# boolsi/boolsi

Hardware: AMD Instinct MI355X
Metric: node-state-updates/s (higher is better)
Workload: dtype u32

## Files before the change

boolsi_amd/csrc/bsx_cascade.cpp:

```cpp
#include <cmath>
#include <cstdio>
#include <cstring>

#include "bsx_attract_host.h"

using namespace bsx;

namespace {
constexpr uint64_t kUnresCap = 1ull << 16;
constexpr uint64_t kNearBytes = 1ull << 32;
}

namespace bsx {

static int mirror_slots_for(bsx_handle h, uint32_t* slots_out) {
    const uint64_t entries = (h->cube_mirror ? 2 : 1) * h->journal_states;
    uint32_t slots = 64;
    while (slots < 2 * entries && slots < h->cache_lds_slots) slots *= 2;
    const size_t fixed = h->shmem + 32 + pool_extra_bytes(h->net.nw);
    while (slots < 4 * entries && slots < h->cache_lds_slots && fixed + (size_t)2 * slots * h->cache_stride <= 80 * 1024) slots *= 2;
    h->mirror_slots = *slots_out = std::min(slots, h->cache_lds_slots);
    if (h->knobs.debug) std::fprintf(stderr, "[bsx] mirror: %llu cycle states cached, %u slots\n", (unsigned long long)h->journal_states, *slots_out);
    return BSX_OK;
}

int lean_mirror_slots(bsx_handle h, uint32_t* slots_out, Totals* tot) {
    uint32_t ignored = 0;
    if (!slots_out) slots_out = &ignored;
    if (!h->journal_stale) return mirror_slots_for(h, slots_out);
    unsigned int known = 0;
    HIPCHK(h, hipMemcpy(&known, h->d_cc_count.p, sizeof(known), hipMemcpyDeviceToHost));
    if (tot) ++tot->syncs;
    known = std::min<unsigned int>(known, kCycleJournalCap);
    h->h_journal.resize(known);
    if (known) HIPCHK(h, hipMemcpy(h->h_journal.data(), h->d_cc_journal.p, known * sizeof(CycleRecord), hipMemcpyDeviceToHost));
    uint64_t states = 0;
    uint32_t taken = 0;
    for (const CycleRecord& r : h->h_journal) {
        if (taken >= (uint32_t)kTagAcc + kLdsAcc) break;
        if (!r.ready || r.length == 0 || r.length > kCycleCacheMaxLen) continue;
        states += r.length;
        ++taken;
    }
    h->journal_states = states;
    h->journal_stale = false;
    return mirror_slots_for(h, slots_out);
}

int ensure_mirror_image(bsx_handle h, AttractParams& P, size_t shmem) {
    if (!h->knobs.mirror_image) { P.mirror_image = nullptr; P.mirror_out = nullptr; return BSX_OK; }
    const size_t words = 4 + (size_t)P.cc.lds_slots * (h->cache_stride / 4);
    if (h->image_n != h->h_journal.size() || h->image_slots != P.cc.lds_slots || h->d_mirror.n < words) {
        HIPCHK(h, h->d_mirror.reserve(words));
        AttractParams B = P;
        B.count = 0;
        B.level_in = nullptr;
        B.mirror_image = nullptr;
        B.mirror_out = h->d_mirror.p;
        HIPCHK(h, launch_attract_pool((int)h->net.nw, (int)h->net.k_mux, h->lut_mode, dim3(1), shmem, h->stream, B));
        h->image_n = h->h_journal.size();
        h->image_slots = P.cc.lds_slots;
    }
    P.mirror_image = h->d_mirror.p;
    P.mirror_out = nullptr;
    return BSX_OK;
}

}

namespace {

int order_cube_digits(bsx_handle h, Cube& c) {
    const uint32_t r = (uint32_t)c.rel.size();
    if (r < 2 || r > 64 || !h->knobs.cube_order) return BSX_OK;
    uint64_t need = 0;
    for (uint32_t q = 0; q < r; ++q) need |= 1ull << c.rel[q];
    if (need & ~h->life_valid) {
        LifetimeParams L{};
        L.net = h->net;
        for (int w = 0; w < kMaxW32; ++w) { L.fixmask[w] = h->sp.fixmask[w]; L.fixval[w] = h->sp.fixval[w]; L.base[w] = c.base[w]; L.free_mask[w] = c.free_mask[w]; }
        L.n_digits = r;
        for (uint32_t q = 0; q < r; ++q) L.node[q] = h->model.any[c.rel[q]];
        HIPCHK(h, h->d_life.reserve(64));
        HIPCHK(h, hipMemsetAsync(h->d_life.p, 0, 64 * sizeof(uint32_t), h->stream));
// ... 201 lines not shown
            }
        }
        const size_t shmem_here = Q.lower_build ? h->shmem + (size_t)B.slots * h->cache_stride + 32 + pool_lower_extra_bytes(nw) : B.shmem;
        hipStream_t const st = i == 0 ? main_st : tail_st;
        HIPCHK(h, launch_attract_pool((int)nw, (int)h->net.k_mux, h->lut_mode, grid, shmem_here, st, Q));
        if (i == 0) HIPCHK(h, hipEventRecord(ev[1], main_st));
        if (i == 0 && side) HIPCHK(h, hipStreamWaitEvent(tail_st, ev[1], 0));
    }
    if (side) {
        HIPCHK(h, hipEventRecord(ev[2], tail_st));
        slot_busy[slot] = ev[2];
    }
    return BSX_OK;
}

int evaluate_chain(bsx_handle h, const CascadeEnv& env, const CascadeShape& sh, const Chain& ch, MergedTable& pass_table,
                   u128& pass_none, u128& pass_ref, int& verdict, uint32_t& lower_to) {
    const AttractParams& P = env.P;
    Totals& tot = env.tot;
    const uint64_t max_t = env.max_t, max_len = env.max_len;
    const uint32_t nw = h->net.nw, rec_words = nw + 3;
    verdict = kChainOk;
    uint64_t n_entries = 0;
    for (uint32_t i = 0; i < ch.top; ++i) {
        const ChainLevel& l = ch.lv[i];
        const Counters& c = h->ctr_seen[ch.ctr_base + i];
        const uint64_t classes = i == 0 ? 1ull << l.k_bits : n_entries << l.k_bits;
        if (i > 0 && n_entries == 0) break;
        tot.steps_exec += c.steps_exec;
        if (h->knobs.debug)
            std::fprintf(stderr, "[bsx] cube 2^%u (%u digits free) at digit value %llu%s: depth %u%s, %u digits here (%u relevant), %llu classes, %llu near a cycle, %llu unresolved\n",
                         ch.c1.a, ch.c1.n_free, (unsigned long long)ch.c1.d_lo, ch.c1.fix_mask ? " [sub-block]" : "", l.depth, i == 0 ? " (top)" : l.per_parent ? " (per parent)" : "", l.k_bits, l.r_here,
                         (unsigned long long)classes, (unsigned long long)c.near_classes, (unsigned long long)c.straggler_classes);
        if (h->knobs.debug && l.per_parent) {
            const LeafProgram& prog = h->h_leaf[ch.index];
            std::fprintf(stderr, "[bsx] per-parent level: kb %u, %u enumerated rules, %u free rules, m %u\n", prog.kb, prog.n_enum, prog.n_free, prog.m);
        }
        if (c.straggler_overflow) { verdict = kChainGiveUp; return BSX_OK; }
        if (c.near_overflow) { verdict = kChainLower; lower_to = l.depth - 1; return BSX_OK; }
        n_entries = c.near_classes;
        {
            double* seen = h->plan.near_seen[i == 0 ? 0 : 1][std::min<uint32_t>(l.depth, kMaxCubeLevels)];
            seen[0] += (double)classes; seen[1] += (double)c.near_classes;
        }
        const uint32_t us = l.unit_shift;
        merge_cube_counters(pass_table, c, us, nw);
        fold_cube_level(c, us, max_t, pass_none, pass_ref);
        const uint64_t n_unres = c.straggler_classes;
        if (!n_unres) continue;
        if (n_unres > kUnresCap) { verdict = kChainGiveUp; return BSX_OK; }
        std::vector<uint32_t> recs(n_unres * rec_words);
        HIPCHK(h, hipMemcpy(recs.data(), h->d_unres.p + (size_t)(ch.ctr_base + i) * kUnresCap * rec_words, recs.size() * 4, hipMemcpyDeviceToHost));
        ++tot.syncs;
        std::vector<uint32_t> st(n_unres * nw);
        for (uint64_t q = 0; q < n_unres; ++q) std::copy(recs.begin() + q * rec_words, recs.begin() + q * rec_words + nw, st.begin() + q * nw);
        DevBuf<uint32_t> d_states;
        DevBuf<ProblemRec32> d_res;
        HIPCHK(h, d_states.upload(st));
        HIPCHK(h, d_res.alloc(n_unres));
        AttractParams S = P;
        S.sp = l.cube.sp;
        S.sp.tp_origin = 0;
        S.count = n_unres;
        S.states = d_states.p;
        S.per_problem = d_res.p;
        S.max_len = BSX_T_INF;
// ... 244 lines not shown
```

boolsi_amd/csrc/bsx_device.h:

```cpp
#pragma once
#include <cstddef>
#include <stdint.h>

namespace bsx {

constexpr int kWave = 64;
constexpr int kBlock = 512;
constexpr int kWavesPerBlock = kBlock / kWave;
constexpr int kPoolBlockThreads = 768;
constexpr uint32_t kPoolCap = 112;
constexpr uint32_t kPoolSlots = 128;
constexpr uint32_t pool_rec_words(uint32_t nw) { return nw + 4; }
constexpr uint32_t kLowerFoundWords = 256;
constexpr int kMaxW32 = 8;
constexpr int kMaxMuxK = 6;
constexpr int kTableSlots = 64;
constexpr uint32_t kStepLimit = 1u << 30;
constexpr uint64_t kDigestSeed = 0xCBF29CE484222325ull;
constexpr uint64_t kDigestPrime = 0x100000001B3ull;
constexpr uint32_t kMaxDepositRuns = 64;

struct DevNet {
    uint32_t n_nodes;
    uint32_t nw;
// ... 45 lines not shown
    uint32_t trajectory_l;
    uint32_t found;
    uint32_t pad;
};

struct alignas(256) Counters {
    unsigned long long cursor;
    unsigned long long steps_ref;
    unsigned long long steps_exec;
    unsigned long long n_none;
    unsigned long long log_cursor;
    unsigned int log_overflow;
    unsigned int step_limit_hits;
    unsigned long long n_stragglers;
    unsigned long long n_cache_resolved;
    unsigned long long straggler_classes;
    unsigned int straggler_overflow;
    unsigned int pad;
    unsigned long long table_inserts;
    unsigned int table_overflow;
    unsigned int near_overflow;
    unsigned long long phase_sum[3];
    unsigned long long phase_max[3];
    unsigned long long acc_cnt[64], acc_sl[64], acc_sl2_lo[64], acc_sl2_hi[64];
    unsigned int acc_len[64];
    unsigned int acc_key[64][kMaxW32];
    unsigned long long fix_cnt[64], fix_sl[64], fix_sl2[64];
    unsigned long long fix_none, fix_ref, fix_capfail;
    unsigned long long near_classes;
    unsigned long long t_first_not, t_last;
    unsigned long long wave_iters;
    unsigned long long service_rounds;
    unsigned long long diag[4];
};

constexpr uint32_t kCycleCacheMaxLen = 64;
constexpr uint32_t kCycleCacheLdsBytes = 16 * 1024;
constexpr uint32_t kCycleJournalCap = 4096;
constexpr uint32_t kCycleClaimSlots = 8192;
constexpr int kTagAcc = 3;
constexpr uint32_t kLdsAcc = 61;
constexpr uint32_t kMergeGroup = 32;
constexpr uint32_t kMergeSlots = 256;
constexpr uint32_t lean_acc_bytes(uint32_t nw) { return (kTagAcc + kLdsAcc) * (8 + 8 + 4 + 4 + 4 * nw) + 16 + kWavesPerBlock * (kMergeSlots + 256); }

struct CycleRecord {
    uint32_t key[kMaxW32];
    uint32_t length;
    uint32_t ready;
};
static_assert(sizeof(CycleRecord) == 40, "CycleRecord layout");

struct CycleCache {
    CycleRecord* journal;
    unsigned int* journal_count;
    unsigned int* claims;
    uint32_t enabled;
    uint32_t lds_slots;
};

struct LevelDesc {
    unsigned long long n_entries;
    unsigned int abort;
    unsigned int pad;
};
constexpr uint32_t kMaxCubeLevels = 16;
constexpr uint32_t kSideStreams = 4;
constexpr uint32_t kMaxChains = 48;
constexpr uint32_t kMaxChainBlocks = 160;
constexpr size_t kLevelDescBytes = 3584;
constexpr size_t kPublishTicketOffset = kLevelDescBytes - 16;
static_assert(sizeof(LevelDesc) * (kMaxChainBlocks + kMaxChains + 1) <= kPublishTicketOffset && kLevelDescBytes % 256 == 0, "descriptor block");

constexpr uint32_t kLeafMaxDeps = 64;
// ... 147 lines not shown
```

boolsi_amd/csrc/bsx_kernels_common.h:

```cpp
#pragma once
#include <hip/hip_runtime.h>
#include <type_traits>
#include "bsx_device.h"

namespace bsx {

__device__ __forceinline__ uint32_t bfi(uint32_t sel, uint32_t a, uint32_t b) {
    uint32_t r;
    asm("v_bfi_b32 %0, %1, %2, %3" : "=v"(r) : "v"(sel), "v"(a), "v"(b));
    return r;
}

#define BSX_KERNARG(Type, name)                                                                          \
    const Type* name = (const Type*)__builtin_amdgcn_kernarg_segment_ptr();                              \
    asm volatile("" : "+s"(name))

__device__ __forceinline__ uint32_t rank_below(uint64_t mask) {
    return __builtin_amdgcn_mbcnt_hi((uint32_t)(mask >> 32), __builtin_amdgcn_mbcnt_lo((uint32_t)mask, 0u));
}

template <int NW>
__device__ __forceinline__ bool eq_words(const uint32_t (&a)[NW], const uint32_t (&b)[NW]) {
    uint32_t d = 0;
#pragma unroll
// ... 285 lines not shown
        if (range == 3) { digit = (uint32_t)(variant % 3); variant /= 3; }
        else { digit = (uint32_t)(variant & 1); variant >>= 1; }
        const int st = digit_state(range, digit);
        if (st >= 0) { put_bit<NW>(pr.fm, node, 1); put_bit<NW>(pr.fv, node, (uint32_t)st); }
    }
    pr.pv_digits = 0;
    pr.tp = sp.tp_origin;
    for (uint32_t j = 0; j < sp.n_pv; ++j) {
        const uint32_t t = sp.pv[3 * j], range = sp.pv[3 * j + 2];
        uint32_t digit;
        if (range == 3) { digit = (uint32_t)(variant % 3); variant /= 3; }
        else { digit = (uint32_t)(variant & 1); variant >>= 1; }
        pr.pv_digits |= (uint64_t)digit << (2 * j);
        if (digit_state(range, digit) >= 0 && t > pr.tp) pr.tp = t;
    }
}

template <int NW>
__device__ __forceinline__ void apply_perturbations(const DevSpace& sp, uint32_t t, uint64_t pv_digits,
                                                    uint32_t (&s)[NW]) {
    if (t <= sp.tp_origin) {
#pragma unroll
        for (int w = 0; w < NW; ++w)
            s[w] = (s[w] & ~sp.sched_clr[t * NW + w]) | sp.sched_set[t * NW + w];
    }
    for (uint32_t j = 0; j < sp.n_pv; ++j) {
        if (sp.pv[3 * j] == t) {
            const int st = digit_state(sp.pv[3 * j + 2], (uint32_t)(pv_digits >> (2 * j)) & 3u);
            if (st >= 0) put_bit<NW>(s, sp.pv[3 * j + 1], (uint32_t)st);
        }
    }
}

template <int NW, int K, int LM>
__device__ __forceinline__ NetView<NW, K, LM> stage_network(const DevNet& net, uint32_t* smem, uint32_t*& smem_free) {
    constexpr bool LDS_LUT = LM != kLutGlobal;
    NetView<NW, K, LM> nv;
    if constexpr (LDS_LUT) {
        if ((uint32_t)(uintptr_t)(__attribute__((address_space(3))) uint32_t*)smem != 0u) __builtin_trap();
    }
    uint32_t* p = smem;
    uint32_t* smasks = p;
    const uint32_t n_masks = (1u << K) * NW;
    for (uint32_t i = threadIdx.x; i < n_masks; i += blockDim.x) smasks[i] = net.masks[i];
    p += (n_masks + 3u) & ~3u;
    if (LDS_LUT) {
        uint32_t* slut = p;
        const uint4* src = reinterpret_cast<const uint4*>(net.lut);
        uint4* dst = reinterpret_cast<uint4*>(slut);
        const uint32_t n4 = net.lut_words >> 2;
        for (uint32_t i = threadIdx.x; i < n4; i += blockDim.x) dst[i] = src[i];
        p += net.lut_words;
        nv.lut = slut;
    } else {
        nv.lut = net.lut;
    }
    __syncthreads();
    nv.masks = smasks;
    if constexpr (NetView<NW, K, LM>::kMasksInRegs) {
#pragma unroll
        for (int i = 0; i < (1 << K) * NW; ++i) nv.mreg[i] = smasks[i];
    } else {
        nv.mreg[0] = 0;
    }
    nv.n_wide = net.n_wide;
    nv.wide_desc = net.wide_desc;
    nv.wide_preds = net.wide_preds;
    nv.wide_tt = net.wide_tt;
    smem_free = p;
    return nv;
}

__device__ __forceinline__ uint32_t digest_ybit(uint32_t t) { return (t * 0x9E3779B1u) >> 31; }
template <int NW>
__device__ __forceinline__ uint64_t digest_fold_words(uint64_t dg, const uint32_t (&s)[NW], uint32_t w64) {
#pragma unroll
    for (int w = 0; w < (NW + 1) / 2; ++w) {
        uint64_t word = s[2 * w];
        if (2 * w + 1 < NW) word |= (uint64_t)s[2 * w + 1] << 32;
        if ((uint32_t)w < w64) dg = (dg ^ word) * kDigestPrime;
    }
    return dg;
}

__device__ __forceinline__ uint64_t bcast64(uint64_t v, int src_lane) {
    const uint32_t lo = __builtin_amdgcn_readlane((uint32_t)v, src_lane);
    const uint32_t hi = __builtin_amdgcn_readlane((uint32_t)(v >> 32), src_lane);
    return ((uint64_t)hi << 32) | lo;
}

__device__ __forceinline__ unsigned long long wave_sum(unsigned long long v) {
#pragma unroll
    for (int off = 32; off >= 1; off >>= 1) {
        const uint32_t lo = __shfl_xor((uint32_t)v, off, 64);
        const uint32_t hi = __shfl_xor((uint32_t)(v >> 32), off, 64);
        v += ((unsigned long long)hi << 32) | lo;
    }
    return v;
}
__device__ __forceinline__ void wave_atomic_add(unsigned long long* dst, unsigned long long v, int lane) {
    const unsigned long long total = wave_sum(v);
    if (lane == 0 && total) atomicAdd(dst, total);
// ... 342 lines not shown
```

boolsi_amd/csrc/bsx_pool_kernel.h:

```cpp
#pragma once
#include "bsx_kernels_common.h"
#include "bsx_leaf.h"

namespace bsx {

constexpr int kPoolBlock = kPoolBlockThreads;
constexpr int kPoolWaves = kPoolBlock / 64;
constexpr uint32_t kPoolGroup = 64;

constexpr int pool_min_waves(int nw) { return nw <= 2 ? 6 : 2; }

#define BSX_RARE_PARAMS(name) BSX_KERNARG(AttractParams, name)

template <int NW>
__device__ __forceinline__ void deposit_runs(const DevSpace& sp, uint64_t d, uint32_t (&s)[NW], uint32_t run_first = 0,
                                             uint32_t run_end = 0xFFFFFFFFu) {
    const uint32_t end = run_end < sp.n_runs ? run_end : sp.n_runs;
    for (uint32_t r = run_first; r < end; ++r) {
        const uint32_t desc = sp.deposit[2 * r], mask = sp.deposit[2 * r + 1];
        const uint32_t piece = ((uint32_t)(d >> (desc & 63u)) & mask) << ((desc >> 16) & 31u);
        const uint32_t word = (desc >> 8) & 7u;
#pragma unroll
        for (int w = 0; w < NW; ++w) s[w] |= (word == (uint32_t)w) ? piece : 0u;
    }
}

template <int NW, int K, int LM, bool CUBE, bool LOWER = false>
__global__ __launch_bounds__(kPoolBlock, pool_min_waves(NW)) void k_attract_pool(const AttractParams P) {
    static_assert(CUBE || !LOWER, "the lower-level build is a cube build");
    extern __shared__ __attribute__((aligned(16))) uint32_t smem[];
    uint32_t* smem_free;
#ifdef BSX_DIAG
    const unsigned long long dbg_t0 = wall_clock64();
#endif
    uint64_t n_items = P.count, chunk_first = P.chunk_first;
    uint32_t chunk = P.chunk;
    if constexpr (CUBE) {
        if (P.level_in) {
            const unsigned long long listed = P.level_in->n_entries;
            n_items = P.level_in->abort ? 0ull : listed << P.entry_shift;
            if constexpr (LOWER) {
                if (P.leaf && n_items) n_items = ((listed + 63ull) & ~63ull) * leaf_parts(P.leaf->m, listed, (uint64_t)gridDim.x * kPoolWaves);
            }
            if (n_items == 0) return;
            const uint64_t n_waves = (uint64_t)gridDim.x * kPoolWaves;
            if (n_items < (1ull << 28)) { chunk_first = ((n_items + n_waves - 1) / n_waves + 63) / 64 * 64; chunk = 0; }
            else { chunk_first = 4096; chunk = 4096; }
            if ((uint64_t)blockIdx.x * chunk_first >= n_items) return;
        }
    }
    if constexpr (CUBE) {
        if (threadIdx.x == 0 && !P.mirror_out) atomicMax(&P.ctr->t_first_not, ~(unsigned long long)wall_clock64());
    }
    const NetView<NW, K, LM> nv = stage_network<NW, K, LM>(P.net, smem, smem_free);
    const uint32_t lane = threadIdx.x & 63, wave = __builtin_amdgcn_readfirstlane(threadIdx.x >> 6);
    const uint32_t tp = P.sp.tp_origin;
    const bool has_warmup = tp != 0;
    const bool counting = CUBE || P.merge >= 2;
    constexpr bool cube = CUBE;
    const int32_t fast_steps = (int32_t)P.fast_steps;
    const uint32_t cmask = P.cc.lds_slots - 1;
    constexpr int S = CacheLayout<NW>::kStride;
    constexpr uint32_t kAccs = (uint32_t)kTagAcc + kLdsAcc;
    constexpr uint32_t R = cube ? NW + 2 : pool_rec_words(NW);
    constexpr uint32_t kCap = cube ? (kPoolCap * pool_rec_words(NW)) / (NW + 2) : kPoolCap;

    uint32_t* lc = smem + (((uint32_t)(smem_free - smem) + 3u) & ~3u);
    const uint32_t lc_words = kCacheHeaderWords + P.cc.lds_slots * S;
    unsigned long long* acc_sl2 = reinterpret_cast<unsigned long long*>(lc + ((lc_words + 1u) & ~1u));
    unsigned long long* acc_sl2h = acc_sl2 + kAccs;
    unsigned long long* acc_sl = acc_sl2h + kAccs;
    unsigned long long* acc_cnt = acc_sl + kAccs;
    uint32_t* lamtab = reinterpret_cast<uint32_t*>(acc_cnt + kAccs);
    uint32_t* keytab = lamtab + kAccs;
    constexpr uint32_t kWaveWords = LOWER ? 0u : kPoolCap * pool_rec_words(NW) + 128 + kPoolSlots / 4;
    constexpr uint32_t kFoundWords = LOWER ? kLowerFoundWords : 0u;
    constexpr uint32_t kLowerCntWords = LOWER ? 2u * kAccs : 0u;
    static_assert(kAccs % 2 == 0 && kWaveWords % 2 == 0, "64-bit LDS atomics need 8-byte aligned tables");
    unsigned long long* wg_ctr = reinterpret_cast<unsigned long long*>(keytab + ((kAccs * NW + 1u) & ~1u));
    uint32_t* midtab = reinterpret_cast<uint32_t*>(wg_ctr + 4);
    uint32_t* wave_base = midtab + 64 * NW + kFoundWords + wave * (kWaveWords + kLowerCntWords);
    typedef volatile uint32_t __attribute__((address_space(3))) lds_vu32;
    typedef volatile uint8_t __attribute__((address_space(3))) lds_vu8;
    lds_vu32* const pool = (lds_vu32*)(__attribute__((address_space(3))) uint32_t*)wave_base;
    lds_vu32* const dd_acc = pool + kPoolCap * pool_rec_words(NW);
    lds_vu8* const dd_ids = (lds_vu8*)(dd_acc + 128);

    uint32_t fm0[NW], fv0[NW];
    uint32_t any_fixed = 0;
#pragma unroll
    for (int w = 0; w < NW; ++w) { fm0[w] = P.sp.fixmask[w]; fv0[w] = P.sp.fixval[w]; any_fixed |= fm0[w]; }
    const bool has_fixed = any_fixed != 0;
    const uint32_t* const image = P.mirror_image;
    if (image) { for (uint32_t i = threadIdx.x; i < lc_words; i += blockDim.x) lc[i] = image[i]; }
    else { for (uint32_t i = threadIdx.x; i < lc_words; i += blockDim.x) lc[i] = 0; }
    for (uint32_t i = threadIdx.x; i < kAccs; i += blockDim.x) { acc_sl2[i] = 0; acc_sl2h[i] = 0; acc_sl[i] = 0; acc_cnt[i] = 0; lamtab[i] = 0; }
    if (threadIdx.x < 4) wg_ctr[threadIdx.x] = 0;
    if constexpr (!LOWER) { dd_acc[2 * lane] = 0; dd_acc[2 * lane + 1] = 0; }
    else { wave_base[lane] = 0; wave_base[64 + lane] = 0; }
    __syncthreads();
    if (!image && threadIdx.x == 0) {
        uint32_t seen = 0, n_states = 0, n_attr = 0;
        cache_pull<NW, K>(P.cc, nv, fm0, fv0, lc, seen, n_states, n_attr, kAccs);
    }
    __syncthreads();
    if (P.mirror_out) {
        for (uint32_t i = threadIdx.x; i < lc_words; i += blockDim.x) P.mirror_out[i] = lc[i];
        return;
    }
    const uint32_t* cbase = lc + kCacheHeaderWords;
    for (uint32_t sl = threadIdx.x; sl < P.cc.lds_slots; sl += blockDim.x) {
        const uint32_t tg = cbase[sl * S + NW] & kTagMask;
        if (tg) {
            lamtab[tg - 1] = cbase[sl * S + NW + 1];
#pragma unroll
            for (int w = 0; w < NW; ++w) keytab[(tg - 1) * NW + w] = cbase[sl * S + NW + 2 + w];
        }
    }
    __syncthreads();
    if constexpr (cube) {
        for (uint32_t i = threadIdx.x; i < 64u; i += blockDim.x) {
            uint32_t m[NW];
#pragma unroll
            for (int w = 0; w < NW; ++w) m[w] = 0;
            deposit_runs<NW>(P.sp, (uint64_t)i << 6, m, 6u, 12u);
#pragma unroll
            for (int w = 0; w < NW; ++w) midtab[i * NW + w] = m[w];
        }
    }
    const uint32_t depth = (cube && P.cube_depth > 1u) ? P.cube_depth : 1u;
    const bool from_entries = cube && P.entries != nullptr;
    if constexpr (cube) {
        if (threadIdx.x == 0) { lc[1] = 0; lc[2] = 0; }
        __syncthreads();
        if (depth == 1u && !has_warmup) {
            constexpr uint32_t kFoundCap = LOWER ? kLowerFoundWords : kCap * R;
            auto inside = [&](uint32_t sl) -> bool {
                const uint32_t* e = cbase + sl * S;
                const uint32_t tw = e[NW];
                if ((tw & kTagMask) == 0 || (tw & kTagRep)) return false;
                uint32_t outside = 0;
#pragma unroll
                for (int w = 0; w < NW; ++w) outside |= (e[w] ^ P.sp.origin[w]) & ~P.cube_free[w];
                return outside == 0;
            };
            lds_vu32* const found0 = (lds_vu32*)(__attribute__((address_space(3))) uint32_t*)(midtab + 64 * NW);
            for (uint32_t sl = threadIdx.x; sl < P.cc.lds_slots; sl += blockDim.x) {
                if (!inside(sl)) continue;
                const uint32_t at = atomicAdd((uint32_t*)(__attribute__((address_space(3))) uint32_t*)&lc[1], 1u);
                if (at < kFoundCap) found0[at] = sl;
            }
            __syncthreads();
            if (threadIdx.x == 0) {
                const uint32_t n_in = lc[1];
                auto add_rep = [&](uint32_t sl) {
                    const uint32_t* e = cbase + sl * S;
                    uint32_t rep[NW], key[NW], differs = 0;
#pragma unroll
                    for (int w = 0; w < NW; ++w) {
                        rep[w] = e[w] & ~P.cube_umask[w];
                        differs |= rep[w] ^ e[w];
                        key[w] = e[NW + 2 + w];
                    }
                    if (differs) cache_insert_lds<NW>(lc, cmask, rep, e[NW + 1], key, (e[NW] & kTagMask) | kTagRep);
                };
                if (n_in <= kFoundCap) {
                    for (uint32_t i = 0; i < n_in; ++i) add_rep(found0[i]);
                } else {
                    for (uint32_t sl = 0; sl < P.cc.lds_slots; ++sl) if (inside(sl)) add_rep(sl);
                }
            }
        }
    }
    __syncthreads();
    const bool t0_lookup = cube && !has_warmup && depth == 1u && __builtin_amdgcn_readfirstlane(lc[1]) != 0;
    uint32_t lane_part[NW];
#pragma unroll
    for (int w = 0; w < NW; ++w) lane_part[w] = 0;
    if constexpr (cube) deposit_runs<NW>(P.sp, (uint64_t)lane, lane_part);
    uint32_t u_hi[NW];
    uint64_t u_hi_tag = ~0ull;
#pragma unroll
    for (int w = 0; w < NW; ++w) u_hi[w] = 0;

    const uint32_t cap_rel = (P.cap_rel_inf || P.max_t - tp >= (kStepLimit / 4)) ? 0xFFFFFFFFu : (uint32_t)(P.max_t - tp);

    using cnt_t = std::conditional_t<CUBE, unsigned long long, uint32_t>;
    uint32_t nexec = 0;
    const uint64_t first_dyn = (uint64_t)gridDim.x * kPoolWaves * chunk_first;
    WaveQueue q{0, 0, chunk != 0 && n_items > first_dyn};
    {
        const uint64_t b = ((uint64_t)wave * gridDim.x + blockIdx.x) * chunk_first;
        if (b < n_items) { q.next = b; q.end = (b + chunk_first < n_items) ? b + chunk_first : n_items; }
    }
    uint32_t head = 0, count = 0;
#ifdef BSX_DIAG
    unsigned long long dbg_iters = 0, dbg_fresh = 0, dbg_fresh_keep = 0, dbg_pool_in = 0, dbg_pool_keep = 0, dbg_merged = 0;
    bool dbg_is_fresh = false;
#endif

    uint32_t ptag = 0;
    auto fresh_state = [&](uint64_t pos, bool lv, uint32_t (&S0)[NW]) {
        if ((pos >> 12) != u_hi_tag) {
            u_hi_tag = pos >> 12;
#pragma unroll
            for (int w = 0; w < NW; ++w) u_hi[w] = P.sp.origin[w];
            deposit_runs<NW>(P.sp, pos & ~0xFFFull, u_hi, 12u);
        }
        const uint32_t mid = (((uint32_t)pos >> 6) & 63u) * NW;
#pragma unroll
        for (int w = 0; w < NW; ++w) S0[w] = u_hi[w] | midtab[mid + w] | lane_part[w];
        if (P.entries) {
            const uint64_t e = (pos + lane) >> P.entry_shift;
            if (lv) {
#pragma unroll
                for (int w = 0; w < NW; ++w) S0[w] |= P.entries[e * (NW + 1) + w];
                ptag = P.entries[e * (NW + 1) + NW];
            }
        }
    };

    uint32_t hit_len = 0;
    auto probe = [&](const uint32_t (&s)[NW], uint32_t& hfull, bool reps = false) -> uint32_t {
        const uint32_t ignore = reps ? 0u : kTagRep;
        hfull = hash_state<NW>(s);
// ... 50 lines not shown
                const unsigned long long up = hi + ((old + lo < old) ? 1ull : 0ull);
                if (up) atomicAdd(&acc_sl2h[tg - 1], up);
            } else {
                atomicAdd(&acc_sl2[tg - 1], wl * traj);
            }
        }
    };

    auto account_fix = [&](uint32_t tagw, uint32_t mu, uint32_t lam, long long sign) {
        BSX_RARE_PARAMS(Pr);
        asm volatile("" : "+v"(mu));
        const uint32_t tg = tagw & kTagMask, traj = tp + mu;
        const bool found = mu <= cap_rel && lam <= cap_rel - mu;
        const bool keep = found && (uint64_t)lam <= Pr->max_len;
        Counters* c = Pr->ctr;
        if (found) atomicAdd(&c->fix_ref, (unsigned long long)(sign * (long long)(traj + lam)));
        else atomicAdd(&c->fix_capfail, (unsigned long long)sign);
        if (!keep) { atomicAdd(&c->fix_none, (unsigned long long)sign); return; }
        c->acc_len[tg - 1] = lam;
#pragma unroll
        for (int w = 0; w < NW; ++w) c->acc_key[tg - 1][w] = keytab[(tg - 1) * NW + w];
        atomicAdd(&c->fix_cnt[tg - 1], (unsigned long long)sign);
        atomicAdd(&c->fix_sl[tg - 1], (unsigned long long)(sign * (long long)traj));
        atomicAdd(&c->fix_sl2[tg - 1], (unsigned long long)(sign * (long long)traj * (long long)traj));
    };

#ifdef BSX_DIAG
    const unsigned long long dbg_t1 = wall_clock64();
#endif
    if constexpr (LOWER) {
        uint32_t* const wave_cnt = wave_base;
        if (P.leaf) {
            const LeafProgram* const L = P.leaf;
            const uint32_t kb = L->kb, n_dep = L->n_dep, m = L->m, n_enum = L->n_enum, n_free = L->n_free;
            uint32_t indep[NW], added[NW];
#pragma unroll
            for (int w = 0; w < NW; ++w) { indep[w] = L->indep[w]; added[w] = L->added[w]; }
            static_assert(sizeof(LeafDep) == 16 && kLeafMaxDeps * 4 <= kLowerFoundWords, "the rules fit the found list's words");
            uint32_t* const dep_lds = midtab + 64 * NW;
            for (uint32_t i = threadIdx.x; i < n_dep * 4u; i += blockDim.x) dep_lds[i] = reinterpret_cast<const uint32_t*>(L->dep)[i];
            __syncthreads();
            if (threadIdx.x == 0) lc[1] = 0;
            for (uint32_t sl0 = 0; sl0 < P.cc.lds_slots; sl0 += blockDim.x) {
                const uint32_t sl = sl0 + threadIdx.x;
                uint32_t ew[NW + 1];
#pragma unroll
                for (int w = 0; w <= NW; ++w) ew[w] = sl < P.cc.lds_slots ? lc[kCacheHeaderWords + sl * S + w] : 0u;
                __syncthreads();
                const bool occ = (ew[NW] & kTagMask) != 0;
                const uint64_t ob = __ballot(occ);
                uint32_t at0 = 0;
                if (lane == 0 && ob) at0 = atomicAdd((uint32_t*)(__attribute__((address_space(3))) uint32_t*)&lc[1], (uint32_t)__popcll(ob));
                const uint32_t at = __builtin_amdgcn_readfirstlane(at0) + rank_below(ob);
                if (occ) {
#pragma unroll
                    for (int w = 0; w <= NW; ++w) lc[kCacheHeaderWords + at * S + w] = ew[w];
                }
            }
            __syncthreads();
            const uint32_t n_occupied = __builtin_amdgcn_readfirstlane(lc[1]);
            const unsigned long long listed = P.level_in->n_entries, listed64 = (listed + 63ull) & ~63ull;
            const uint32_t parts = leaf_parts(m, listed, (uint64_t)gridDim.x * kPoolWaves);
            const uint32_t children_per_part = leaf_children_per_part(kb, m, parts);
            for (;;) {
                if (q.next == q.end) {
                    if (!q.more) break;
                    BSX_RARE_PARAMS(Pr);
                    const uint64_t b = first_dyn + grab_chunk(&Pr->ctr->cursor, chunk, (int)lane);
                    if (b >= n_items) { q.more = false; continue; }
                    q.next = b; q.end = (b + chunk < n_items) ? b + chunk : n_items;
                }
                const uint64_t avail = q.end - q.next;
                const uint32_t n = avail < 64u ? (uint32_t)avail : 64u;
                const uint32_t part = (uint32_t)(q.next / listed64);
                const unsigned long long pbase = q.next - (unsigned long long)part * listed64;
                const bool lv = lane < n && pbase + lane < listed;
                uint32_t Sp[NW], Y[NW], tagp = 0;
#pragma unroll
                for (int w = 0; w < NW; ++w) { Sp[w] = 0; Y[w] = 0; }
                if (lv) {
                    const uint32_t* ent = P.entries + (pbase + lane) * (NW + 1);
#pragma unroll
                    for (int w = 0; w < NW; ++w) Sp[w] = ent[w];
                    tagp = ent[NW];
                    net_step<NW, K>(nv, Sp, fm0, fv0, Y, has_fixed);
                    nexec += part == 0u ? 1u : 0u;
                }
                q.next += n;
                uint32_t hits = 0;
                for (uint32_t sl = 0; sl < n_occupied; ++sl) {
                    const uint32_t* e = cbase + sl * S;
                    const uint32_t tagw = __builtin_amdgcn_readfirstlane(e[NW]);
                    if ((tagw & kTagMask) == 0) continue;
// ... 430 lines not shown
            ri -= ri >= kCap ? kCap : 0u;
            const uint32_t r = ri * R;
            if constexpr (cube) {
                const uint32_t packed = mhi | ((uint32_t)(t + 256) << 17);
                if constexpr (NW == 2) {
                    typedef volatile bsx_u32x4 __attribute__((address_space(3))) lds_v4;
                    bsx_u32x4 v;
                    v.x = A[0]; v.y = A[1]; v.z = mlo; v.w = packed;
                    *(lds_v4*)(pool + r) = v;
                } else {
#pragma unroll
                    for (int w = 0; w < NW; ++w) pool[r + w] = A[w];
                    pool[r + NW] = mlo; pool[r + NW + 1] = packed;
                }
            } else if constexpr (NW % 2 == 0) {
                typedef volatile bsx_u32x2 __attribute__((address_space(3))) lds_v2;
                lds_v2* rec = (lds_v2*)(pool + r);
#pragma unroll
                for (int w = 0; w < NW; w += 2) { bsx_u32x2 v; v.x = A[w]; v.y = A[w + 1]; rec[w / 2] = v; }
                bsx_u32x2 b0, b1;
                b0.x = base; b0.y = mlo; b1.x = mhi; b1.y = (uint32_t)t;
                rec[NW / 2] = b0; rec[NW / 2 + 1] = b1;
            } else {
#pragma unroll
                for (int w = 0; w < NW; ++w) pool[r + w] = A[w];
                pool[r + NW] = base; pool[r + NW + 1] = mlo; pool[r + NW + 2] = mhi; pool[r + NW + 3] = (uint32_t)t;
            }
        }
        count += (uint32_t)__popcll(keepers);
        __builtin_amdgcn_fence(__ATOMIC_RELEASE, "wavefront");
        __builtin_amdgcn_wave_barrier();
    }

    __syncthreads();
#ifdef BSX_DIAG
    const unsigned long long dbg_t2 = wall_clock64();
#endif
    static_assert(kAccs == 64, "one lane per accumulator");
    if (wave == 0) {
        const uint32_t a = lane;
        const unsigned long long cn = acc_cnt[a];
        const uint64_t nb = __ballot(cn != 0);
        if (nb) {
            unsigned long long at0 = 0;
            if (!cube && lane == 0) at0 = atomicAdd(&P.ctr->log_cursor, (unsigned long long)__popcll(nb));
            const unsigned long long at = bcast64(at0, 0) + rank_below(nb);
            if (cn) {
                const unsigned long long sl = acc_sl[a];
                if constexpr (cube) {
                    Counters* c = P.ctr;
                    atomicAdd(&c->acc_cnt[a], cn);
                    atomicAdd(&c->acc_sl[a], sl);
                    const unsigned long long lo = acc_sl2[a];
                    const unsigned long long old = atomicAdd(&c->acc_sl2_lo[a], lo);
                    const unsigned long long up = acc_sl2h[a] + ((old + lo < old) ? 1ull : 0ull);
                    if (up) atomicAdd(&c->acc_sl2_hi[a], up);
                    c->acc_len[a] = lamtab[a];
#pragma unroll
                    for (int w = 0; w < NW; ++w) c->acc_key[a][w] = keytab[a * NW + w];
                } else if (at < P.log_cap) {
                    LogRec r;
#pragma unroll
                    for (int w = 0; w < kMaxW32; ++w) r.key[w] = 0;
#pragma unroll
                    for (int w = 0; w < NW; ++w) r.key[w] = keytab[a * NW + w];
                    r.length = lamtab[a]; r.pad = 0; r.count = cn; r.sum_l = sl; r.sum_l2_lo = acc_sl2[a]; r.sum_l2_hi = acc_sl2h[a];
                    P.log[at] = r;
                } else {
                    atomicOr(&P.ctr->log_overflow, 1u);
                }
                atomicAdd(&wg_ctr[2], sl + cn * lamtab[a]);
            }
        }
    }
#ifdef BSX_DIAG
    if (lane == 0) {
        atomicAdd(&P.ctr->wave_iters, dbg_iters); atomicAdd(&P.ctr->service_rounds, dbg_fresh);
        atomicAdd(&P.ctr->diag[0], dbg_fresh_keep); atomicAdd(&P.ctr->diag[1], dbg_pool_in);
        atomicAdd(&P.ctr->diag[2], dbg_pool_keep); atomicAdd(&P.ctr->diag[3], dbg_merged);
    }
    if (threadIdx.x == 0) {
        const unsigned long long dbg_t3 = wall_clock64();
        atomicAdd(&P.ctr->phase_sum[0], dbg_t1 - dbg_t0); atomicMax(&P.ctr->phase_max[0], dbg_t1 - dbg_t0);
        atomicAdd(&P.ctr->phase_sum[1], dbg_t2 - dbg_t1); atomicMax(&P.ctr->phase_max[1], dbg_t2 - dbg_t1);
        atomicAdd(&P.ctr->phase_sum[2], dbg_t3 - dbg_t2); atomicMax(&P.ctr->phase_max[2], dbg_t3 - dbg_t2);
    }
#endif
    {
        const unsigned long long w_exec = wave_sum((unsigned long long)nexec);
        if (lane == 0 && w_exec) atomicAdd(&wg_ctr[3], w_exec);
    }
    __builtin_amdgcn_fence(__ATOMIC_RELEASE, "workgroup");
    __builtin_amdgcn_s_barrier();
    __builtin_amdgcn_fence(__ATOMIC_ACQUIRE, "workgroup");
    if (threadIdx.x == 0) {
        if constexpr (cube) {
            BSX_RARE_PARAMS(Pr);
            if (Pr->level_out) {
                const uint32_t listed = lc[2];
                const uint32_t mine = listed < Pr->near_cap ? listed : (uint32_t)Pr->near_cap;
                lc[1] = mine ? (uint32_t)atomicAdd(&Pr->level_out->n_entries, (unsigned long long)mine) : 0u;
                if (listed) atomicAdd(&P.ctr->near_classes, (unsigned long long)listed);
                if (listed > Pr->near_cap) {
                    atomicOr(&Pr->level_out->abort, 1u);
                    atomicOr(&P.ctr->near_overflow, 1u);
                }
            }
        }
        const unsigned long long ref = wg_ctr[2] + (P.cap_rel_inf ? 0ull : wg_ctr[1] * P.max_t);
        if (ref) atomicAdd(&P.ctr->steps_ref, ref);
        if (wg_ctr[3]) atomicAdd(&P.ctr->steps_exec, wg_ctr[3]);
        if (wg_ctr[0]) atomicAdd(&P.ctr->n_none, wg_ctr[0]);
        if constexpr (cube) atomicMax(&P.ctr->t_last, (unsigned long long)wall_clock64());
    }
    if constexpr (cube) {
        BSX_RARE_PARAMS(Pr);
        if (Pr->level_out) {
            __syncthreads();
            const uint32_t listed = lc[2], base = lc[1];
            const uint64_t words = (uint64_t)(listed < Pr->near_cap ? listed : (uint32_t)Pr->near_cap) * (NW + 1);
            const uint32_t* src = Pr->near + (uint64_t)blockIdx.x * Pr->near_cap * (NW + 1);
            uint32_t* dst = Pr->near_list + (uint64_t)base * (NW + 1);
            for (uint64_t i = threadIdx.x; i < words; i += kPoolBlock) dst[i] = src[i];
        }
    }
}

template <int NW, int K, int LM>
__global__ __launch_bounds__(1024) void k_digit_lifetimes(const LifetimeParams P) {
    extern __shared__ __attribute__((aligned(16))) uint32_t smem[];
    uint32_t* smem_free;
    const NetView<NW, K, LM> nv = stage_network<NW, K, LM>(P.net, smem, smem_free);
    const uint32_t digit = threadIdx.x / kLifeTrials, trial = threadIdx.x % kLifeTrials;
    if (digit >= P.n_digits) return;
    uint32_t fm[NW], fv[NW], x[NW], y[NW];
    uint32_t any_fixed = 0;
    const uint32_t node = P.node[digit];
#pragma unroll
    for (int w = 0; w < NW; ++w) {
        fm[w] = P.fixmask[w]; fv[w] = P.fixval[w]; any_fixed |= fm[w];
        uint32_t rnd = (trial * 0x9E3779B1u + (uint32_t)w * 0x85EBCA6Bu + 0x27D4EB2Fu) * 0xC2B2AE35u;
// ... 123 lines not shown
```

Before: 16280 billion.

## Overlap network, cache image and leaf-table staging in the pool kernel prologue

Splits network staging into begin/LUT/end phases so the LDS LUT copy, the mirror-image tables and a precompacted list of occupied cache slots are loaded together in one batched vectorised copy before a single barrier. The mirror image now also stores accumulator tables and a compacted occupied-slot list. This removes several per-workgroup barriers and the LDS compaction loop from the per-parent leaf path. The epilogue reorders the near-list atomic reservation ahead of the accumulator flush and packs the first chunk assignment per block. The cost is a more complex image layout, more registers for staged loads and subtle ordering between phases.

Result: no change. 16530 billion (median of 2 runs) (+1.6%).

```diff
diff --git a/boolsi_amd/csrc/bsx_cascade.cpp b/boolsi_amd/csrc/bsx_cascade.cpp
--- a/boolsi_amd/csrc/bsx_cascade.cpp
+++ b/boolsi_amd/csrc/bsx_cascade.cpp
@@ -49,7 +49,7 @@
 
 int ensure_mirror_image(bsx_handle h, AttractParams& P, size_t shmem) {
     if (!h->knobs.mirror_image) { P.mirror_image = nullptr; P.mirror_out = nullptr; return BSX_OK; }
-    const size_t words = 4 + (size_t)P.cc.lds_slots * (h->cache_stride / 4);
+    const size_t words = (size_t)pool_image_words(h->net.nw, P.cc.lds_slots, h->cache_stride / 4) + pool_image_list_words(P.cc.lds_slots, h->cache_stride / 4);
     if (h->image_n != h->h_journal.size() || h->image_slots != P.cc.lds_slots || h->d_mirror.n < words) {
         HIPCHK(h, h->d_mirror.reserve(words));
         AttractParams B = P;
@@ -317,6 +317,10 @@
             std::fprintf(stderr, "[bsx] cube 2^%u (%u digits free) at digit value %llu%s: depth %u%s, %u digits here (%u relevant), %llu classes, %llu near a cycle, %llu unresolved\n",
                          ch.c1.a, ch.c1.n_free, (unsigned long long)ch.c1.d_lo, ch.c1.fix_mask ? " [sub-block]" : "", l.depth, i == 0 ? " (top)" : l.per_parent ? " (per parent)" : "", l.k_bits, l.r_here,
                          (unsigned long long)classes, (unsigned long long)c.near_classes, (unsigned long long)c.straggler_classes);
+        if (h->knobs.debug && c.phase_wgs)
+            std::fprintf(stderr, "[bsx]   phases: %llu workgroups; staging / prologue / loop / epilogue, us: mean %.1f / %.1f / %.1f / %.1f, slowest (prologue / loop / epilogue) %.1f / %.1f / %.1f\n",
+                         (unsigned long long)c.phase_wgs, c.phase_stage / 100.0 / c.phase_wgs, c.phase_sum[0] / 100.0 / c.phase_wgs, c.phase_sum[1] / 100.0 / c.phase_wgs,
+                         c.phase_sum[2] / 100.0 / c.phase_wgs, c.phase_max[0] / 100.0, c.phase_max[1] / 100.0, c.phase_max[2] / 100.0);
         if (h->knobs.debug && l.per_parent) {
             const LeafProgram& prog = h->h_leaf[ch.index];
             std::fprintf(stderr, "[bsx] per-parent level: kb %u, %u enumerated rules, %u free rules, m %u\n", prog.kb, prog.n_enum, prog.n_free, prog.m);
diff --git a/boolsi_amd/csrc/bsx_device.h b/boolsi_amd/csrc/bsx_device.h
--- a/boolsi_amd/csrc/bsx_device.h
+++ b/boolsi_amd/csrc/bsx_device.h
@@ -101,14 +101,20 @@
     unsigned long long wave_iters;
     unsigned long long service_rounds;
     unsigned long long diag[4];
+    unsigned long long phase_stage;
+    unsigned long long phase_wgs;
 };
 
 constexpr uint32_t kCycleCacheMaxLen = 64;
 constexpr uint32_t kCycleCacheLdsBytes = 16 * 1024;
 constexpr uint32_t kCycleJournalCap = 4096;
 constexpr uint32_t kCycleClaimSlots = 8192;
+constexpr uint32_t pool_image_list_words(uint32_t slots, uint32_t stride_words) { return 4u + (slots / 2u) * stride_words; }
 constexpr int kTagAcc = 3;
 constexpr uint32_t kLdsAcc = 61;
+constexpr uint32_t pool_image_words(uint32_t nw, uint32_t slots, uint32_t stride_words) {
+    return 4u + slots * stride_words + (kTagAcc + kLdsAcc) * (4u * 2u + 1u) + (((kTagAcc + kLdsAcc) * nw + 1u) & ~1u) + 8u;
+}
 constexpr uint32_t kMergeGroup = 32;
 constexpr uint32_t kMergeSlots = 256;
 constexpr uint32_t lean_acc_bytes(uint32_t nw) { return (kTagAcc + kLdsAcc) * (8 + 8 + 4 + 4 + 4 * nw) + 16 + kWavesPerBlock * (kMergeSlots + 256); }
diff --git a/boolsi_amd/csrc/bsx_kernels_common.h b/boolsi_amd/csrc/bsx_kernels_common.h
--- a/boolsi_amd/csrc/bsx_kernels_common.h
+++ b/boolsi_amd/csrc/bsx_kernels_common.h
@@ -341,8 +341,33 @@
     }
 }
 
+struct StageJob {
+    bsx_u32x4* dst;
+    const bsx_u32x4* src;
+    uint32_t n4;
+};
+template <int A, int B, int C>
+__device__ __forceinline__ void stage_copy3(const StageJob& a, const StageJob& b, const StageJob& c) {
+    bsx_u32x4 va[A] = {}, vb[B] = {}, vc[C] = {};
+#pragma unroll
+    for (int j = 0; j < A; ++j) { const uint32_t i = threadIdx.x + j * blockDim.x; if (i < a.n4) va[j] = a.src[i]; }
+#pragma unroll
+    for (int j = 0; j < B; ++j) { const uint32_t i = threadIdx.x + j * blockDim.x; if (i < b.n4) vb[j] = b.src[i]; }
+#pragma unroll
+    for (int j = 0; j < C; ++j) { const uint32_t i = threadIdx.x + j * blockDim.x; if (i < c.n4) vc[j] = c.src[i]; }
+#pragma unroll
+    for (int j = 0; j < A; ++j) { const uint32_t i = threadIdx.x + j * blockDim.x; if (i < a.n4) a.dst[i] = va[j]; }
+#pragma unroll
+    for (int j = 0; j < B; ++j) { const uint32_t i = threadIdx.x + j * blockDim.x; if (i < b.n4) b.dst[i] = vb[j]; }
+#pragma unroll
+    for (int j = 0; j < C; ++j) { const uint32_t i = threadIdx.x + j * blockDim.x; if (i < c.n4) c.dst[i] = vc[j]; }
+    for (uint32_t i = threadIdx.x + A * blockDim.x; i < a.n4; i += blockDim.x) a.dst[i] = a.src[i];
+    for (uint32_t i = threadIdx.x + B * blockDim.x; i < b.n4; i += blockDim.x) b.dst[i] = b.src[i];
+    for (uint32_t i = threadIdx.x + C * blockDim.x; i < c.n4; i += blockDim.x) c.dst[i] = c.src[i];
+}
+
 template <int NW, int K, int LM>
-__device__ __forceinline__ NetView<NW, K, LM> stage_network(const DevNet& net, uint32_t* smem, uint32_t*& smem_free) {
+__device__ __forceinline__ NetView<NW, K, LM> stage_network_begin(const DevNet& net, uint32_t* smem, uint32_t*& smem_free) {
     constexpr bool LDS_LUT = LM != kLutGlobal;
     NetView<NW, K, LM> nv;
     if constexpr (LDS_LUT) {
@@ -354,29 +379,41 @@
     for (uint32_t i = threadIdx.x; i < n_masks; i += blockDim.x) smasks[i] = net.masks[i];
     p += (n_masks + 3u) & ~3u;
     if (LDS_LUT) {
-        uint32_t* slut = p;
-        const uint4* src = reinterpret_cast<const uint4*>(net.lut);
-        uint4* dst = reinterpret_cast<uint4*>(slut);
-        const uint32_t n4 = net.lut_words >> 2;
-        for (uint32_t i = threadIdx.x; i < n4; i += blockDim.x) dst[i] = src[i];
+        nv.lut = p;
         p += net.lut_words;
-        nv.lut = slut;
     } else {
         nv.lut = net.lut;
     }
-    __syncthreads();
     nv.masks = smasks;
-    if constexpr (NetView<NW, K, LM>::kMasksInRegs) {
-#pragma unroll
-        for (int i = 0; i < (1 << K) * NW; ++i) nv.mreg[i] = smasks[i];
-    } else {
-        nv.mreg[0] = 0;
-    }
+    nv.mreg[0] = 0;
     nv.n_wide = net.n_wide;
     nv.wide_desc = net.wide_desc;
     nv.wide_preds = net.wide_preds;
     nv.wide_tt = net.wide_tt;
     smem_free = p;
+    return nv;
+}
+template <int NW, int K, int LM>
+__device__ __forceinline__ void stage_network_lut(const DevNet& net, const NetView<NW, K, LM>& nv, const StageJob& more = StageJob{nullptr, nullptr, 0},
+                                                  const StageJob& more2 = StageJob{nullptr, nullptr, 0}) {
+    constexpr bool LDS_LUT = LM != kLutGlobal;
+    const uint32_t n4 = LDS_LUT ? net.lut_words >> 2 : 0u;
+    const StageJob lut{reinterpret_cast<bsx_u32x4*>(const_cast<uint32_t*>(nv.lut)), reinterpret_cast<const bsx_u32x4*>(net.lut), n4};
+    stage_copy3<3, 1, 1>(lut, more, more2);
+}
+template <int NW, int K, int LM>
+__device__ __forceinline__ void stage_network_end(NetView<NW, K, LM>& nv) {
+    if constexpr (NetView<NW, K, LM>::kMasksInRegs) {
+#pragma unroll
+        for (int i = 0; i < (1 << K) * NW; ++i) nv.mreg[i] = nv.masks[i];
+    }
+}
+template <int NW, int K, int LM>
+__device__ __forceinline__ NetView<NW, K, LM> stage_network(const DevNet& net, uint32_t* smem, uint32_t*& smem_free) {
+    NetView<NW, K, LM> nv = stage_network_begin<NW, K, LM>(net, smem, smem_free);
+    stage_network_lut<NW, K, LM>(net, nv);
+    __syncthreads();
+    stage_network_end<NW, K, LM>(nv);
     return nv;
 }
 
diff --git a/boolsi_amd/csrc/bsx_pool_kernel.h b/boolsi_amd/csrc/bsx_pool_kernel.h
--- a/boolsi_amd/csrc/bsx_pool_kernel.h
+++ b/boolsi_amd/csrc/bsx_pool_kernel.h
@@ -35,24 +35,34 @@
 #endif
     uint64_t n_items = P.count, chunk_first = P.chunk_first;
     uint32_t chunk = P.chunk;
+    bool packed = false;
+    uint32_t n_listed = 0, leaf_m = 0;
+    if constexpr (LOWER) {
+        if (P.leaf) {
+            leaf_m = P.leaf->m;
+            n_listed = P.mirror_image[pool_image_words(NW, P.cc.lds_slots, CacheLayout<NW>::kStride) + 3u];
+            if (n_listed > P.cc.lds_slots / 2u) n_listed = P.cc.lds_slots / 2u;
+        }
+    }
     if constexpr (CUBE) {
         if (P.level_in) {
             const unsigned long long listed = P.level_in->n_entries;
             n_items = P.level_in->abort ? 0ull : listed << P.entry_shift;
             if constexpr (LOWER) {
-                if (P.leaf && n_items) n_items = ((listed + 63ull) & ~63ull) * leaf_parts(P.leaf->m, listed, (uint64_t)gridDim.x * kPoolWaves);
+                if (P.leaf && n_items) n_items = ((listed + 63ull) & ~63ull) * leaf_parts(leaf_m, listed, (uint64_t)gridDim.x * kPoolWaves);
             }
             if (n_items == 0) return;
             const uint64_t n_waves = (uint64_t)gridDim.x * kPoolWaves;
             if (n_items < (1ull << 28)) { chunk_first = ((n_items + n_waves - 1) / n_waves + 63) / 64 * 64; chunk = 0; }
             else { chunk_first = 4096; chunk = 4096; }
-            if ((uint64_t)blockIdx.x * chunk_first >= n_items) return;
+            packed = chunk == 0;
+            if (packed ? (uint64_t)blockIdx.x * kPoolWaves * chunk_first >= n_items : (uint64_t)blockIdx.x * chunk_first >= n_items) return;
         }
     }
     if constexpr (CUBE) {
         if (threadIdx.x == 0 && !P.mirror_out) atomicMax(&P.ctr->t_first_not, ~(unsigned long long)wall_clock64());
     }
-    const NetView<NW, K, LM> nv = stage_network<NW, K, LM>(P.net, smem, smem_free);
+    NetView<NW, K, LM> nv = stage_network_begin<NW, K, LM>(P.net, smem, smem_free);
     const uint32_t lane = threadIdx.x & 63, wave = __builtin_amdgcn_readfirstlane(threadIdx.x >> 6);
     const uint32_t tp = P.sp.tp_origin;
     const bool has_warmup = tp != 0;
@@ -92,32 +102,28 @@
     for (int w = 0; w < NW; ++w) { fm0[w] = P.sp.fixmask[w]; fv0[w] = P.sp.fixval[w]; any_fixed |= fm0[w]; }
     const bool has_fixed = any_fixed != 0;
     const uint32_t* const image = P.mirror_image;
-    if (image) { for (uint32_t i = threadIdx.x; i < lc_words; i += blockDim.x) lc[i] = image[i]; }
-    else { for (uint32_t i = threadIdx.x; i < lc_words; i += blockDim.x) lc[i] = 0; }
-    for (uint32_t i = threadIdx.x; i < kAccs; i += blockDim.x) { acc_sl2[i] = 0; acc_sl2h[i] = 0; acc_sl[i] = 0; acc_cnt[i] = 0; lamtab[i] = 0; }
-    if (threadIdx.x < 4) wg_ctr[threadIdx.x] = 0;
+    static_assert(kCacheHeaderWords == 4 && kAccs == 64, "bsx_device.h: pool_image_words describes this layout");
+    const uint32_t img_words = pool_image_words(NW, P.cc.lds_slots, S);
+    bool per_parent = false;
+    if constexpr (LOWER) per_parent = P.leaf != nullptr;
+    uint32_t* const dep_lds = midtab + 64 * NW;
+    if (image && per_parent) {
+        const StageJob tables{reinterpret_cast<bsx_u32x4*>(lc + lc_words), reinterpret_cast<const bsx_u32x4*>(image + lc_words), (img_words - lc_words) >> 2};
+        const StageJob list{reinterpret_cast<bsx_u32x4*>(lc), reinterpret_cast<const bsx_u32x4*>(image + img_words), (kCacheHeaderWords + n_listed * S) >> 2};
+        stage_network_lut<NW, K, LM>(P.net, nv, tables, list);
+        if constexpr (LOWER) {
+            static_assert(sizeof(LeafDep) == 16 && kLeafMaxDeps * 4 <= kLowerFoundWords, "the rules fit the found list's words");
+            const uint32_t dep_words = P.leaf->n_dep * 4u;
+            for (uint32_t i = threadIdx.x; i < dep_words && i < kLowerFoundWords; i += blockDim.x) dep_lds[i] = reinterpret_cast<const uint32_t*>(P.leaf->dep)[i];
+        }
+    } else if (image) {
+        stage_network_lut<NW, K, LM>(P.net, nv, StageJob{reinterpret_cast<bsx_u32x4*>(lc), reinterpret_cast<const bsx_u32x4*>(image), img_words >> 2});
+    } else {
+        stage_network_lut<NW, K, LM>(P.net, nv);
+        for (uint32_t i = threadIdx.x; i < img_words; i += blockDim.x) lc[i] = 0;
+    }
     if constexpr (!LOWER) { dd_acc[2 * lane] = 0; dd_acc[2 * lane + 1] = 0; }
     else { wave_base[lane] = 0; wave_base[64 + lane] = 0; }
-    __syncthreads();
-    if (!image && threadIdx.x == 0) {
-        uint32_t seen = 0, n_states = 0, n_attr = 0;
-        cache_pull<NW, K>(P.cc, nv, fm0, fv0, lc, seen, n_states, n_attr, kAccs);
-    }
-    __syncthreads();
-    if (P.mirror_out) {
-        for (uint32_t i = threadIdx.x; i < lc_words; i += blockDim.x) P.mirror_out[i] = lc[i];
-        return;
-    }
-    const uint32_t* cbase = lc + kCacheHeaderWords;
-    for (uint32_t sl = threadIdx.x; sl < P.cc.lds_slots; sl += blockDim.x) {
-        const uint32_t tg = cbase[sl * S + NW] & kTagMask;
-        if (tg) {
-            lamtab[tg - 1] = cbase[sl * S + NW + 1];
-#pragma unroll
-            for (int w = 0; w < NW; ++w) keytab[(tg - 1) * NW + w] = cbase[sl * S + NW + 2 + w];
-        }
-    }
-    __syncthreads();
     if constexpr (cube) {
         for (uint32_t i = threadIdx.x; i < 64u; i += blockDim.x) {
             uint32_t m[NW];
@@ -128,11 +134,46 @@
             for (int w = 0; w < NW; ++w) midtab[i * NW + w] = m[w];
         }
     }
+    __syncthreads();
+    stage_network_end<NW, K, LM>(nv);
+#ifdef BSX_DIAG
+    const unsigned long long dbg_ts = wall_clock64();
+#endif
+    const uint32_t* cbase = lc + kCacheHeaderWords;
+    if (!image) {
+        if (threadIdx.x == 0) {
+            uint32_t seen = 0, n_states = 0, n_attr = 0;
+            cache_pull<NW, K>(P.cc, nv, fm0, fv0, lc, seen, n_states, n_attr, kAccs);
+        }
+        __syncthreads();
+        for (uint32_t sl = threadIdx.x; sl < P.cc.lds_slots; sl += blockDim.x) {
+            const uint32_t tg = cbase[sl * S + NW] & kTagMask;
+            if (tg) {
+                lamtab[tg - 1] = cbase[sl * S + NW + 1];
+#pragma unroll
+                for (int w = 0; w < NW; ++w) keytab[(tg - 1) * NW + w] = cbase[sl * S + NW + 2 + w];
+            }
+        }
+        __syncthreads();
+    }
+    if (P.mirror_out) {
+        for (uint32_t i = threadIdx.x; i < img_words; i += blockDim.x) P.mirror_out[i] = lc[i];
+        __syncthreads();
+        uint32_t* const list_out = P.mirror_out + img_words;
+        for (uint32_t sl = threadIdx.x; sl < P.cc.lds_slots; sl += blockDim.x) {
+            if ((cbase[sl * S + NW] & kTagMask) == 0) continue;
+            const uint32_t at = atomicAdd((uint32_t*)(__attribute__((address_space(3))) uint32_t*)&lc[3], 1u);
+            if (at >= P.cc.lds_slots / 2u) continue;
+#pragma unroll
+            for (int w = 0; w < S; ++w) list_out[kCacheHeaderWords + at * S + w] = w == NW ? cbase[sl * S + w] & ~kTagCont : cbase[sl * S + w];
+        }
+        __syncthreads();
+        if (threadIdx.x < (uint32_t)kCacheHeaderWords) list_out[threadIdx.x] = threadIdx.x == 0 ? lc[0] : threadIdx.x == 3 ? lc[3] : 0u;
+        return;
+    }
     const uint32_t depth = (cube && P.cube_depth > 1u) ? P.cube_depth : 1u;
     const bool from_entries = cube && P.entries != nullptr;
     if constexpr (cube) {
-        if (threadIdx.x == 0) { lc[1] = 0; lc[2] = 0; }
-        __syncthreads();
         if (depth == 1u && !has_warmup) {
             constexpr uint32_t kFoundCap = LOWER ? kLowerFoundWords : kCap * R;
             auto inside = [&](uint32_t sl) -> bool {
@@ -145,6 +186,23 @@
                 return outside == 0;
             };
             lds_vu32* const found0 = (lds_vu32*)(__attribute__((address_space(3))) uint32_t*)(midtab + 64 * NW);
+            if (per_parent) {
+                for (uint32_t i = threadIdx.x; i < n_listed; i += blockDim.x) {
+                    if (!inside(i)) continue;
+                    const uint32_t* e = cbase + i * S;
+                    uint32_t rep[NW], differs = 0;
+#pragma unroll
+                    for (int w = 0; w < NW; ++w) { rep[w] = e[w] & ~P.cube_umask[w]; differs |= rep[w] ^ e[w]; }
+                    if (!differs) continue;
+                    const uint32_t at = n_listed + atomicAdd((uint32_t*)(__attribute__((address_space(3))) uint32_t*)&lc[1], 1u);
+                    if (at >= P.cc.lds_slots) continue;
+                    uint32_t* r = lc + kCacheHeaderWords + at * S;
+#pragma unroll
+                    for (int w = 0; w < NW; ++w) { r[w] = rep[w]; r[NW + 2 + w] = e[NW + 2 + w]; }
+                    r[NW + 1] = e[NW + 1];
+                    r[NW] = (e[NW] & kTagMask) | kTagRep;
+                }
+            } else {
             for (uint32_t sl = threadIdx.x; sl < P.cc.lds_slots; sl += blockDim.x) {
                 if (!inside(sl)) continue;
                 const uint32_t at = atomicAdd((uint32_t*)(__attribute__((address_space(3))) uint32_t*)&lc[1], 1u);
@@ -170,9 +228,10 @@
                     for (uint32_t sl = 0; sl < P.cc.lds_slots; ++sl) if (inside(sl)) add_rep(sl);
                 }
             }
-        }
-    }
-    __syncthreads();
+            }
+            __syncthreads();
+        }
+    }
     const bool t0_lookup = cube && !has_warmup && depth == 1u && __builtin_amdgcn_readfirstlane(lc[1]) != 0;
     uint32_t lane_part[NW];
 #pragma unroll
@@ -190,7 +249,7 @@
     const uint64_t first_dyn = (uint64_t)gridDim.x * kPoolWaves * chunk_first;
     WaveQueue q{0, 0, chunk != 0 && n_items > first_dyn};
     {
-        const uint64_t b = ((uint64_t)wave * gridDim.x + blockIdx.x) * chunk_first;
+        const uint64_t b = (packed ? (uint64_t)blockIdx.x * kPoolWaves + wave : (uint64_t)wave * gridDim.x + blockIdx.x) * chunk_first;
         if (b < n_items) { q.next = b; q.end = (b + chunk_first < n_items) ? b + chunk_first : n_items; }
     }
     uint32_t head = 0, count = 0;
@@ -307,33 +366,12 @@
         uint32_t* const wave_cnt = wave_base;
         if (P.leaf) {
             const LeafProgram* const L = P.leaf;
-            const uint32_t kb = L->kb, n_dep = L->n_dep, m = L->m, n_enum = L->n_enum, n_free = L->n_free;
+            const uint32_t kb = L->kb, m = L->m, n_enum = L->n_enum, n_free = L->n_free;
             uint32_t indep[NW], added[NW];
 #pragma unroll
             for (int w = 0; w < NW; ++w) { indep[w] = L->indep[w]; added[w] = L->added[w]; }
-            static_assert(sizeof(LeafDep) == 16 && kLeafMaxDeps * 4 <= kLowerFoundWords, "the rules fit the found list's words");
-            uint32_t* const dep_lds = midtab + 64 * NW;
-            for (uint32_t i = threadIdx.x; i < n_dep * 4u; i += blockDim.x) dep_lds[i] = reinterpret_cast<const uint32_t*>(L->dep)[i];
-            __syncthreads();
-            if (threadIdx.x == 0) lc[1] = 0;
-            for (uint32_t sl0 = 0; sl0 < P.cc.lds_slots; sl0 += blockDim.x) {
-                const uint32_t sl = sl0 + threadIdx.x;
-                uint32_t ew[NW + 1];
-#pragma unroll
-                for (int w = 0; w <= NW; ++w) ew[w] = sl < P.cc.lds_slots ? lc[kCacheHeaderWords + sl * S + w] : 0u;
-                __syncthreads();
-                const bool occ = (ew[NW] & kTagMask) != 0;
-                const uint64_t ob = __ballot(occ);
-                uint32_t at0 = 0;
-                if (lane == 0 && ob) at0 = atomicAdd((uint32_t*)(__attribute__((address_space(3))) uint32_t*)&lc[1], (uint32_t)__popcll(ob));
-                const uint32_t at = __builtin_amdgcn_readfirstlane(at0) + rank_below(ob);
-                if (occ) {
-#pragma unroll
-                    for (int w = 0; w <= NW; ++w) lc[kCacheHeaderWords + at * S + w] = ew[w];
-                }
-            }
-            __syncthreads();
-            const uint32_t n_occupied = __builtin_amdgcn_readfirstlane(lc[1]);
+            uint32_t n_occupied = n_listed + __builtin_amdgcn_readfirstlane(lc[1]);
+            n_occupied = n_occupied < P.cc.lds_slots ? n_occupied : P.cc.lds_slots;
             const unsigned long long listed = P.level_in->n_entries, listed64 = (listed + 63ull) & ~63ull;
             const uint32_t parts = leaf_parts(m, listed, (uint64_t)gridDim.x * kPoolWaves);
             const uint32_t children_per_part = leaf_children_per_part(kb, m, parts);
@@ -830,10 +868,32 @@
         __builtin_amdgcn_wave_barrier();
     }
 
-    __syncthreads();
+    {
+        const unsigned long long w_exec = wave_sum((unsigned long long)nexec);
+        if (lane == 0 && w_exec) atomicAdd(&wg_ctr[3], w_exec);
+    }
+    __builtin_amdgcn_fence(__ATOMIC_RELEASE, "workgroup");
+    __builtin_amdgcn_s_barrier();
+    __builtin_amdgcn_fence(__ATOMIC_ACQUIRE, "workgroup");
 #ifdef BSX_DIAG
     const unsigned long long dbg_t2 = wall_clock64();
 #endif
+    uint32_t seg_base = 0;
+    if constexpr (cube) {
+        if (threadIdx.x == 0) {
+            BSX_RARE_PARAMS(Pr);
+            if (Pr->level_out) {
+                const uint32_t listed = lc[2];
+                const uint32_t mine = listed < Pr->near_cap ? listed : (uint32_t)Pr->near_cap;
+                if (mine) seg_base = (uint32_t)atomicAdd(&Pr->level_out->n_entries, (unsigned long long)mine);
+                if (listed) atomicAdd(&P.ctr->near_classes, (unsigned long long)listed);
+                if (listed > Pr->near_cap) {
+                    atomicOr(&Pr->level_out->abort, 1u);
+                    atomicOr(&P.ctr->near_overflow, 1u);
+                }
+            }
+        }
+    }
     static_assert(kAccs == 64, "one lane per accumulator");
     if (wave == 0) {
         const uint32_t a = lane;
@@ -882,29 +942,13 @@
         atomicAdd(&P.ctr->phase_sum[0], dbg_t1 - dbg_t0); atomicMax(&P.ctr->phase_max[0], dbg_t1 - dbg_t0);
         atomicAdd(&P.ctr->phase_sum[1], dbg_t2 - dbg_t1); atomicMax(&P.ctr->phase_max[1], dbg_t2 - dbg_t1);
         atomicAdd(&P.ctr->phase_sum[2], dbg_t3 - dbg_t2); atomicMax(&P.ctr->phase_max[2], dbg_t3 - dbg_t2);
-    }
-#endif
-    {
-        const unsigned long long w_exec = wave_sum((unsigned long long)nexec);
-        if (lane == 0 && w_exec) atomicAdd(&wg_ctr[3], w_exec);
-    }
-    __builtin_amdgcn_fence(__ATOMIC_RELEASE, "workgroup");
-    __builtin_amdgcn_s_barrier();
-    __builtin_amdgcn_fence(__ATOMIC_ACQUIRE, "workgroup");
+        atomicAdd(&P.ctr->phase_stage, dbg_ts - dbg_t0); atomicAdd(&P.ctr->phase_wgs, 1ull);
+    }
+#endif
+    __builtin_amdgcn_fence(__ATOMIC_ACQ_REL, "wavefront");
+    __builtin_amdgcn_wave_barrier();
     if (threadIdx.x == 0) {
-        if constexpr (cube) {
-            BSX_RARE_PARAMS(Pr);
-            if (Pr->level_out) {
-                const uint32_t listed = lc[2];
-                const uint32_t mine = listed < Pr->near_cap ? listed : (uint32_t)Pr->near_cap;
-                lc[1] = mine ? (uint32_t)atomicAdd(&Pr->level_out->n_entries, (unsigned long long)mine) : 0u;
-                if (listed) atomicAdd(&P.ctr->near_classes, (unsigned long long)listed);
-                if (listed > Pr->near_cap) {
-                    atomicOr(&Pr->level_out->abort, 1u);
-                    atomicOr(&P.ctr->near_overflow, 1u);
-                }
-            }
-        }
+        if constexpr (cube) lc[1] = seg_base;
         const unsigned long long ref = wg_ctr[2] + (P.cap_rel_inf ? 0ull : wg_ctr[1] * P.max_t);
         if (ref) atomicAdd(&P.ctr->steps_ref, ref);
         if (wg_ctr[3]) atomicAdd(&P.ctr->steps_exec, wg_ctr[3]);
```
